# SobeyMIL/MVOC

Measured on AMD Instinct MI355X. Metric: UNet3D denoising steps/sec, 16x512^2 frames, inversion+compose, higher is better.
Workload: dtype f16

## Files before the change

### include/mvoc_hip.h

```cpp
#ifndef MVOC_HIP_H
#define MVOC_HIP_H

#include <stddef.h>
#include <stdint.h>

#ifdef __cplusplus
extern "C" {
#endif

#define MVOC_VERSION 100

int mvoc_version(void);
const char* mvoc_last_error(void);

enum { MVOC_A_PLAIN = 0, MVOC_A_CONV3X3 = 1, MVOC_A_TEMPORAL3 = 2 };
enum { MVOC_ACT_NONE = 0, MVOC_ACT_GEGLU = 1, MVOC_ACT_SILU = 2, MVOC_ACT_GELU = 3 };

typedef struct mvoc_gemm_desc {
  const void* a;
  const void* a2;
  const void* w;
  void* out;
  const void* bias;
  const void* rowadd;
  const void* resid;
  int64_t m, n, k;
  int32_t n_store;
  int32_t ldo, ldr, ld_rowadd, rowadd_div;
  int32_t a_mode;
  int32_t lda, lda2;
  int32_t c1;
  int32_t cin;
  int32_t nimg, hout, wout, hsrc, wsrc, stride, upsample, hup, wup;
  int32_t frames, hw;
  int32_t act;
  int32_t tile;
  int32_t split_k;
  void* workspace;
  size_t workspace_bytes;
  const void* ln_rowsum;
  const void* ln_bias;
  float ln_eps;
  int32_t pad_mode;
  const void* ln_stats;
  void* chan_sums;
  void* row_moments;
  int32_t row_moments_ld;
  int32_t concurrency;
  int32_t k_order;
} mvoc_gemm_desc;

int mvoc_gemm_f16(const mvoc_gemm_desc* d, void* stream);
int mvoc_gemm_chan_sums_written(void);
int mvoc_gemm_row_moments_written(void);
int mvoc_row_stats_from_moments_f32(const void* moments, int64_t rows, int32_t ld, int32_t n, int32_t tile_w, float eps,
                                    void* out_stats, void* stream);
size_t mvoc_gemm_workspace_bytes(int64_t m, int64_t n, int64_t k);

typedef struct mvoc_attn_desc {
  const void *q, *k, *v;
  void* out;
  int64_t q_bs, q_ts, k_bs, k_ts, v_bs, v_ts, o_bs, o_ts;
  int32_t nbatch, heads, tq, tk, kv_bdiv;
  int32_t head_dim, causal;
  float scale;
  const void* v2;
  void* out2;
  int32_t pipelined;
} mvoc_attn_desc;

int mvoc_flash_attn_f16(const mvoc_attn_desc* d, void* stream);
typedef struct mvoc_tattn_desc {
  const void *q, *k, *v;
  void* out;
  int64_t q_bs, q_ps, q_ts, k_bs, k_ps, k_ts, v_bs, v_ps, v_ts, o_bs, o_ps, o_ts;
  int32_t nsample, hw, heads, frames;
} mvoc_tattn_desc;
int mvoc_temporal_attn_f16(const mvoc_tattn_desc* d, void* stream);

typedef struct mvoc_xs_desc {
  const void* x;
  const void* wp;
  const void* resid;
  void* out;
  int64_t m;
  int32_t n, k, n_store, ldo, ldr, act, normalize;
  float ln_eps;
  int64_t wp_set_rows;
} mvoc_xs_desc;
int mvoc_xs_linear_f16(const mvoc_xs_desc* d, void* stream);


typedef struct mvoc_tfused_desc {
  const void* x;
  const void* wp;
  const void* ln_rowsum;
  const void* ln_bias;
  void* out;
  int32_t nsample, frames, hw, c, heads;
  float ln_eps;
} mvoc_tfused_desc;
int mvoc_temporal_qkv_attn_f16(const mvoc_tfused_desc* d, void* stream);

typedef struct mvoc_gn_desc {
  const void* x;
  const void* x2;
  const void* gamma;
  const void* beta;
  void* out;
  void* workspace;
  size_t workspace_bytes;
  int32_t nsample, rows_per_sample, c, c1, groups, silu;
  float eps;
  const void* chan_sums;
  const void* chan_sums2;
} mvoc_gn_desc;
size_t mvoc_groupnorm_workspace_bytes(int32_t nsample, int32_t rows_per_sample, int32_t c, int32_t groups);
int mvoc_groupnorm_f16(const mvoc_gn_desc* d, void* stream);
int mvoc_groupnorm_fold_xs_f16(const mvoc_gn_desc* d, const void* w, const void* bias, int32_t n, int32_t k, void* wp_sets,
                               void* stream);

int mvoc_groupnorm_moments_f16(const mvoc_gn_desc* d, void* moments, void* stream);
int mvoc_groupnorm_apply_moments_f16(const mvoc_gn_desc* d, const void* parts, int32_t nparts, void* stream);

int mvoc_row_stats_f16(const void* x, void* stats, int64_t rows, int32_t c, float eps, void* stream);

int mvoc_layernorm_f16(const void* x, const void* gamma, const void* beta, void* out, int64_t rows, int32_t c,
                       float eps, void* stream);

typedef struct mvoc_pnp_desc {
  void* x;
  void* x2;
  const void* masks;
  int64_t chunk_stride, f_stride, p_stride;
  int32_t nobj, frames, height, width, channels, mask_h, mask_w, base_chunk0;
  int32_t ndst;
} mvoc_pnp_desc;
int mvoc_pnp_blend_scatter_tokens(const mvoc_pnp_desc* d, void* stream);
int mvoc_pnp_blend_scatter_nchw(const mvoc_pnp_desc* d, void* stream);
int mvoc_pnp_blend_scatter_tokens_mapped(const mvoc_pnp_desc* d, int32_t nsrc, const int32_t* obj_chunk, void* stream);
int mvoc_pnp_blend_scatter_nchw_mapped(const mvoc_pnp_desc* d, int32_t nsrc, const int32_t* obj_chunk, void* stream);
int mvoc_pnp_blend_scatter_tokens_variants(const mvoc_pnp_desc* d, int32_t nsrc, const int32_t* obj_chunk, int32_t nvar,
                                           void* stream);
int mvoc_pnp_blend_scatter_nchw_variants(const mvoc_pnp_desc* d, int32_t nsrc, const int32_t* obj_chunk, int32_t nvar,
                                         void* stream);
int mvoc_pnp_blend_scatter_tokens_variants_sel(const mvoc_pnp_desc* d, int32_t nsrc, const int32_t* obj_chunk, int32_t nvar,
                                               uint32_t active, void* stream);
int mvoc_pnp_blend_scatter_nchw_variants_sel(const mvoc_pnp_desc* d, int32_t nsrc, const int32_t* obj_chunk, int32_t nvar,
                                             uint32_t active, void* stream);
int mvoc_pnp_blend_scatter_tokens_placed(const mvoc_pnp_desc* d, int32_t nsrc, const int32_t* obj_chunk, int32_t nvar,
                                         uint32_t active, const int32_t* place, void* stream);
int mvoc_pnp_blend_scatter_nchw_placed(const mvoc_pnp_desc* d, int32_t nsrc, const int32_t* obj_chunk, int32_t nvar,
                                       uint32_t active, const int32_t* place, void* stream);
int mvoc_pnp_blend_scatter_tokens_placed_variants(const mvoc_pnp_desc* d, int32_t nsrc, const int32_t* obj_chunk, int32_t nvar,
                                                  uint32_t active, const int32_t* place, void* stream);
int mvoc_pnp_blend_scatter_nchw_placed_variants(const mvoc_pnp_desc* d, int32_t nsrc, const int32_t* obj_chunk, int32_t nvar,
                                                uint32_t active, const int32_t* place, void* stream);
int mvoc_shift_planes_f16(const void* src, void* dst, int32_t nplane, int32_t frames, int32_t h, int32_t w,
                          const int32_t* offsets, void* stream);
int mvoc_pnp_blend_scatter_tokens_resampled(const mvoc_pnp_desc* d, int32_t nsrc, const int32_t* obj_chunk, int32_t nvar,
                                            uint32_t active, const int32_t* maps, void* stream);
int mvoc_pnp_blend_scatter_nchw_resampled(const mvoc_pnp_desc* d, int32_t nsrc, const int32_t* obj_chunk, int32_t nvar,
                                          uint32_t active, const int32_t* maps, void* stream);
int mvoc_pnp_blend_scatter_tokens_resampled_variants(const mvoc_pnp_desc* d, int32_t nsrc, const int32_t* obj_chunk, int32_t nvar,
                                                     uint32_t active, const int32_t* maps, void* stream);
int mvoc_pnp_blend_scatter_nchw_resampled_variants(const mvoc_pnp_desc* d, int32_t nsrc, const int32_t* obj_chunk, int32_t nvar,
                                                   uint32_t active, const int32_t* maps, void* stream);
int mvoc_gather_planes_f16(const void* src, void* dst, int32_t nplane, int32_t frames, int32_t h, int32_t w,
                           const int32_t* maps, void* stream);

int mvoc_ddim_step_f16(const void* x, const void* v_uncond, const void* v_cond, const float* coef_dev, void* out,
                       int64_t n, void* stream);
int mvoc_latent_fusion_f16(const void* latents, const void* bg, const void* objs, const void* masks, void* out,
                           int32_t nobj, int64_t n, double mix_ratio, int32_t obj_random_noise_fusion, void* stream);
int mvoc_ddim_step_variants_f16(const void* x, const void* v_uncond, const void* v_cond, const float* coef_dev, void* out,
                                int64_t n_per, int32_t nvar, void* stream);
int mvoc_latent_fusion_variants_f16(const void* latents, const void* bg, const void* objs, const void* masks, void* out,
                                    int32_t nobj, int64_t n_per, int32_t nvar, double mix_ratio,
                                    int32_t obj_random_noise_fusion, void* stream);

int mvoc_timestep_embedding_f16(const float* t_dev, int32_t nb, int32_t dim, void* out, void* stream);
int mvoc_act_f16(const void* x, void* out, int64_t n, int32_t act, void* stream);
int mvoc_add_f16(const void* a, const void* b, void* out, int64_t n, void* stream);
int mvoc_conv3x3_small_f16(const void* x, const void* w, const void* bias, void* out, int32_t nimg, int32_t h,
                           int32_t wd, int32_t cin, int32_t cout, int32_t stride, int32_t silu, void* stream);
int mvoc_adaptive_avgpool_f16(const void* x, void* out, int32_t nimg, int32_t h, int32_t w, int32_t c, int32_t oh,
                              int32_t ow, void* stream);
int mvoc_ncfhw_to_tokens_f16(const void* x, void* out, int32_t b, int32_t c, int32_t f, int32_t hw, int32_t ldo,
                             int32_t coff, void* stream);
int mvoc_tokens_to_ncfhw_f16(const void* x, void* out, int32_t b, int32_t c, int32_t f, int32_t hw, int32_t ld,
                             void* stream);
int mvoc_temporal_encoder4_f16(const void* x, const void* params, void* out, int32_t b, int32_t f, int32_t hw,
                               int32_t ldo, int32_t coff, void* stream);

int mvoc_conv1x1_small_f16(const void* x, const void* w, const void* bias, void* out, int64_t rows, int32_t cin,
                           int32_t cout, void* stream);
int mvoc_softmax_rows_f16(void* x, int64_t rows, int32_t cols, void* stream);
int mvoc_gaussian_sample_f16(const void* mean, const void* logvar, const void* noise, void* out, int64_t n, void* stream);
int mvoc_scale_f16(const void* x, void* out, int64_t n, double scale, void* stream);
int mvoc_image_to_tokens_f16(const void* x, void* out, int32_t n, int32_t c, int32_t hw, void* stream);
int mvoc_tokens_to_image_f16(const void* x, void* out, int32_t n, int32_t c, int32_t hw, int32_t ld, void* stream);

int mvoc_mask_resize_u8(const void* in, void* tmp, void* out, int32_t n, int32_t H, int32_t W, int32_t h, int32_t w,
                        const int32_t* bounds_h, const int32_t* kk_h, int32_t ksize_h, const int32_t* bounds_v,
                        const int32_t* kk_v, int32_t ksize_v, void* stream);
int mvoc_mask_finish(const void* v, void* float_mask, void* bool_mask, int64_t n, void* stream);

int mvoc_clip_patches_f16(const void* pixels, void* out, int32_t nimg, int32_t size, int32_t patch, int32_t kpad, void* stream);
int mvoc_clip_embed_f16(const void* table, const int32_t* ids, const void* cls, const void* pos, void* out, int64_t rows,
                        int32_t t, int32_t c, void* stream);

int mvoc_permute_rows_f16(const void* x, void* out, const int64_t* dims4, const int64_t* strides4, int32_t c, void* stream);
int mvoc_comm_unique_id(void* id128);
int mvoc_comm_init(const void* id128, int32_t rank, int32_t world, void** comm);
int mvoc_comm_destroy(void* comm);
int mvoc_allgather_frames(void* comm, const void* send, void* recv, size_t bytes_per_rank, void* stream);
int mvoc_alltoall_frames(void* comm, const void* send, void* recv, size_t bytes_per_peer, void* stream);

enum { MVOC_FAM_GEMM = 0, MVOC_FAM_FLASH = 1, MVOC_FAM_TATTN = 2, MVOC_FAM_GN = 3, MVOC_FAM_LN = 4, MVOC_FAM_PNP = 5,
       MVOC_FAM_MISC = 6, MVOC_FAM_TFUSED = 7, MVOC_FAM_COUNT = 8 };
int mvoc_prof_enable(int on);
int mvoc_prof_collect(double* ms_per_family, int64_t* launches_per_family, double* flops_or_bytes_per_family);
int mvoc_prof_reset(void);
int mvoc_delay_us(int64_t us, void* stream);

#ifdef __cplusplus
}
#endif
#endif
```

### mvoc_amd/_ffi.py

```python
import ctypes as C
import os

import torch

_HERE = os.path.dirname(os.path.abspath(__file__))
LIB_PATH = os.environ.get("MVOC_HIP_LIB") or os.path.join(_HERE, "libmvoc_hip.so")

ABI_VERSION = 100

A_PLAIN, A_CONV3X3, A_TEMPORAL3 = 0, 1, 2
ACT_NONE, ACT_GEGLU, ACT_SILU, ACT_GELU = 0, 1, 2, 3
FAMILIES = ("gemm", "flash_attn", "temporal_attn", "groupnorm", "layernorm", "pnp", "misc", "temporal_fused")

vp, i32, i64, f32, f64, sz = C.c_void_p, C.c_int32, C.c_int64, C.c_float, C.c_double, C.c_size_t


class GemmDesc(C.Structure):
    _fields_ = [("a", vp), ("a2", vp), ("w", vp), ("out", vp), ("bias", vp), ("rowadd", vp), ("resid", vp),
                ("m", i64), ("n", i64), ("k", i64), ("n_store", i32), ("ldo", i32), ("ldr", i32), ("ld_rowadd", i32),
                ("rowadd_div", i32), ("a_mode", i32), ("lda", i32), ("lda2", i32), ("c1", i32), ("cin", i32),
                ("nimg", i32), ("hout", i32), ("wout", i32), ("hsrc", i32), ("wsrc", i32), ("stride", i32),
                ("upsample", i32), ("hup", i32), ("wup", i32), ("frames", i32), ("hw", i32), ("act", i32), ("tile", i32),
                ("split_k", i32), ("workspace", vp), ("workspace_bytes", sz), ("ln_rowsum", vp), ("ln_bias", vp),
                ("ln_eps", f32), ("pad_mode", i32), ("ln_stats", vp), ("chan_sums", vp), ("row_moments", vp),
                ("row_moments_ld", i32), ("concurrency", i32), ("k_order", i32)]


class AttnDesc(C.Structure):
    _fields_ = [("q", vp), ("k", vp), ("v", vp), ("out", vp),
                ("q_bs", i64), ("q_ts", i64), ("k_bs", i64), ("k_ts", i64), ("v_bs", i64), ("v_ts", i64),
                ("o_bs", i64), ("o_ts", i64),
                ("nbatch", i32), ("heads", i32), ("tq", i32), ("tk", i32), ("kv_bdiv", i32),
                ("head_dim", i32), ("causal", i32), ("scale", C.c_float), ("v2", vp), ("out2", vp), ("pipelined", i32)]


class TAttnDesc(C.Structure):
    _fields_ = [("q", vp), ("k", vp), ("v", vp), ("out", vp),
                ("q_bs", i64), ("q_ps", i64), ("q_ts", i64), ("k_bs", i64), ("k_ps", i64), ("k_ts", i64),
                ("v_bs", i64), ("v_ps", i64), ("v_ts", i64), ("o_bs", i64), ("o_ps", i64), ("o_ts", i64),
                ("nsample", i32), ("hw", i32), ("heads", i32), ("frames", i32)]


class GnDesc(C.Structure):
    _fields_ = [("x", vp), ("x2", vp), ("gamma", vp), ("beta", vp), ("out", vp), ("workspace", vp),
                ("workspace_bytes", sz), ("nsample", i32), ("rows_per_sample", i32), ("c", i32), ("c1", i32),
                ("groups", i32), ("silu", i32), ("eps", f32), ("chan_sums", vp), ("chan_sums2", vp)]


class TFusedDesc(C.Structure):
    _fields_ = [("x", vp), ("wp", vp), ("ln_rowsum", vp), ("ln_bias", vp), ("out", vp), ("nsample", i32), ("frames", i32),
                ("hw", i32), ("c", i32), ("heads", i32), ("ln_eps", f32)]


class XsDesc(C.Structure):
    _fields_ = [("x", vp), ("wp", vp), ("resid", vp), ("out", vp), ("m", i64),
                ("n", i32), ("k", i32), ("n_store", i32), ("ldo", i32), ("ldr", i32), ("act", i32), ("normalize", i32),
                ("ln_eps", C.c_float), ("wp_set_rows", i64)]


class PnpDesc(C.Structure):
    _fields_ = [("x", vp), ("x2", vp), ("masks", vp), ("chunk_stride", i64), ("f_stride", i64), ("p_stride", i64),
                ("nobj", i32), ("frames", i32), ("height", i32), ("width", i32), ("channels", i32), ("mask_h", i32),
                ("mask_w", i32), ("base_chunk0", i32), ("ndst", i32)]


SIGNATURES = {
    "mvoc_version": (i32, []),
    "mvoc_last_error": (C.c_char_p, []),
    "mvoc_gemm_f16": (i32, [C.POINTER(GemmDesc), vp]),
    "mvoc_gemm_workspace_bytes": (sz, [i64, i64, i64]),
    "mvoc_gemm_chan_sums_written": (i32, []),
    "mvoc_gemm_row_moments_written": (i32, []),
    "mvoc_row_stats_from_moments_f32": (i32, [vp, i64, i32, i32, i32, f32, vp, vp]),
    "mvoc_flash_attn_f16": (i32, [C.POINTER(AttnDesc), vp]),
    "mvoc_temporal_attn_f16": (i32, [C.POINTER(TAttnDesc), vp]),
    "mvoc_temporal_qkv_attn_f16": (i32, [C.POINTER(TFusedDesc), vp]),
    "mvoc_xs_linear_f16": (i32, [C.POINTER(XsDesc), vp]),
    "mvoc_groupnorm_workspace_bytes": (sz, [i32, i32, i32, i32]),
    "mvoc_groupnorm_f16": (i32, [C.POINTER(GnDesc), vp]),
    "mvoc_groupnorm_fold_xs_f16": (i32, [C.POINTER(GnDesc), vp, vp, i32, i32, vp, vp]),
    "mvoc_groupnorm_moments_f16": (i32, [C.POINTER(GnDesc), vp, vp]),
    "mvoc_groupnorm_apply_moments_f16": (i32, [C.POINTER(GnDesc), vp, i32, vp]),
    "mvoc_layernorm_f16": (i32, [vp, vp, vp, vp, i64, i32, f32, vp]),
    "mvoc_row_stats_f16": (i32, [vp, vp, i64, i32, f32, vp]),
    "mvoc_pnp_blend_scatter_tokens": (i32, [C.POINTER(PnpDesc), vp]),
    "mvoc_pnp_blend_scatter_nchw": (i32, [C.POINTER(PnpDesc), vp]),
    "mvoc_pnp_blend_scatter_tokens_mapped": (i32, [C.POINTER(PnpDesc), i32, C.POINTER(i32), vp]),
    "mvoc_pnp_blend_scatter_nchw_mapped": (i32, [C.POINTER(PnpDesc), i32, C.POINTER(i32), vp]),
    "mvoc_pnp_blend_scatter_tokens_variants": (i32, [C.POINTER(PnpDesc), i32, C.POINTER(i32), i32, vp]),
    "mvoc_pnp_blend_scatter_nchw_variants": (i32, [C.POINTER(PnpDesc), i32, C.POINTER(i32), i32, vp]),
    "mvoc_pnp_blend_scatter_tokens_variants_sel": (i32, [C.POINTER(PnpDesc), i32, C.POINTER(i32), i32, C.c_uint32, vp]),
    "mvoc_pnp_blend_scatter_nchw_variants_sel": (i32, [C.POINTER(PnpDesc), i32, C.POINTER(i32), i32, C.c_uint32, vp]),
    "mvoc_pnp_blend_scatter_tokens_placed": (i32, [C.POINTER(PnpDesc), i32, C.POINTER(i32), i32, C.c_uint32, vp, vp]),
    "mvoc_pnp_blend_scatter_nchw_placed": (i32, [C.POINTER(PnpDesc), i32, C.POINTER(i32), i32, C.c_uint32, vp, vp]),
    "mvoc_pnp_blend_scatter_tokens_placed_variants": (i32, [C.POINTER(PnpDesc), i32, C.POINTER(i32), i32, C.c_uint32, vp, vp]),
    "mvoc_pnp_blend_scatter_nchw_placed_variants": (i32, [C.POINTER(PnpDesc), i32, C.POINTER(i32), i32, C.c_uint32, vp, vp]),
    "mvoc_shift_planes_f16": (i32, [vp, vp, i32, i32, i32, i32, vp, vp]),
    "mvoc_pnp_blend_scatter_tokens_resampled": (i32, [C.POINTER(PnpDesc), i32, C.POINTER(i32), i32, C.c_uint32, vp, vp]),
    "mvoc_pnp_blend_scatter_nchw_resampled": (i32, [C.POINTER(PnpDesc), i32, C.POINTER(i32), i32, C.c_uint32, vp, vp]),
    "mvoc_pnp_blend_scatter_tokens_resampled_variants": (i32, [C.POINTER(PnpDesc), i32, C.POINTER(i32), i32, C.c_uint32, vp, vp]),
    "mvoc_pnp_blend_scatter_nchw_resampled_variants": (i32, [C.POINTER(PnpDesc), i32, C.POINTER(i32), i32, C.c_uint32, vp, vp]),
    "mvoc_gather_planes_f16": (i32, [vp, vp, i32, i32, i32, i32, vp, vp]),
    "mvoc_ddim_step_f16": (i32, [vp, vp, vp, vp, vp, i64, vp]),
    "mvoc_latent_fusion_f16": (i32, [vp, vp, vp, vp, vp, i32, i64, f64, i32, vp]),
    "mvoc_ddim_step_variants_f16": (i32, [vp, vp, vp, vp, vp, i64, i32, vp]),
    "mvoc_latent_fusion_variants_f16": (i32, [vp, vp, vp, vp, vp, i32, i64, i32, f64, i32, vp]),
    "mvoc_timestep_embedding_f16": (i32, [vp, i32, i32, vp, vp]),
    "mvoc_act_f16": (i32, [vp, vp, i64, i32, vp]),
    "mvoc_add_f16": (i32, [vp, vp, vp, i64, vp]),
    "mvoc_conv3x3_small_f16": (i32, [vp, vp, vp, vp, i32, i32, i32, i32, i32, i32, i32, vp]),
    "mvoc_adaptive_avgpool_f16": (i32, [vp, vp, i32, i32, i32, i32, i32, i32, vp]),
    "mvoc_ncfhw_to_tokens_f16": (i32, [vp, vp, i32, i32, i32, i32, i32, i32, vp]),
    "mvoc_tokens_to_ncfhw_f16": (i32, [vp, vp, i32, i32, i32, i32, i32, vp]),
    "mvoc_temporal_encoder4_f16": (i32, [vp, vp, vp, i32, i32, i32, i32, i32, vp]),
    "mvoc_conv1x1_small_f16": (i32, [vp, vp, vp, vp, i64, i32, i32, vp]),
    "mvoc_softmax_rows_f16": (i32, [vp, i64, i32, vp]),
    "mvoc_gaussian_sample_f16": (i32, [vp, vp, vp, vp, i64, vp]),
    "mvoc_scale_f16": (i32, [vp, vp, i64, f64, vp]),
    "mvoc_image_to_tokens_f16": (i32, [vp, vp, i32, i32, i32, vp]),
    "mvoc_tokens_to_image_f16": (i32, [vp, vp, i32, i32, i32, i32, vp]),
    "mvoc_mask_resize_u8": (i32, [vp, vp, vp, i32, i32, i32, i32, i32, vp, vp, i32, vp, vp, i32, vp]),
    "mvoc_mask_finish": (i32, [vp, vp, vp, i64, vp]),
    "mvoc_permute_rows_f16": (i32, [vp, vp, C.POINTER(i64), C.POINTER(i64), i32, vp]),
    "mvoc_clip_patches_f16": (i32, [vp, vp, i32, i32, i32, i32, vp]),
    "mvoc_clip_embed_f16": (i32, [vp, vp, vp, vp, vp, i64, i32, i32, vp]),
    "mvoc_comm_unique_id": (i32, [vp]),
    "mvoc_comm_init": (i32, [vp, i32, i32, C.POINTER(vp)]),
    "mvoc_comm_destroy": (i32, [vp]),
    "mvoc_allgather_frames": (i32, [vp, vp, vp, sz, vp]),
    "mvoc_alltoall_frames": (i32, [vp, vp, vp, sz, vp]),
    "mvoc_prof_enable": (i32, [i32]),
    "mvoc_prof_collect": (i32, [C.POINTER(f64), C.POINTER(i64), C.POINTER(f64)]),
    "mvoc_prof_reset": (i32, []),
    "mvoc_delay_us": (i32, [i64, vp]),
}


def _load():
    if not os.path.exists(LIB_PATH):
        raise ImportError(
            f"{LIB_PATH} is missing: build it with `python -m mvoc_amd.build` (hipcc --offload-arch=gfx950). "
            "mvoc_amd has no CPU / PyTorch fallback path.")
    lib = C.CDLL(LIB_PATH)
    for name, (res, args) in SIGNATURES.items():
        fn = getattr(lib, name)
        fn.restype = res
        fn.argtypes = args
    if lib.mvoc_version() != ABI_VERSION:
        raise ImportError(f"{LIB_PATH} has mvoc_version() {lib.mvoc_version()}, these bindings need {ABI_VERSION}: rebuild it "
                          "with `python -m mvoc_amd.build`")
    return lib


lib = _load()


_DEBUG_SYNC = bool(os.environ.get("MVOC_DEBUG_SYNC"))


def check(rc, what=""):
    if rc != 0:
        raise RuntimeError(f"libmvoc_hip {what} failed ({rc}): {lib.mvoc_last_error().decode()}")
    if _DEBUG_SYNC:
        print(f"[mvoc] {what}", flush=True)
        torch.cuda.synchronize()
```

### mvoc_amd/csrc/xslin.hip

```cpp
#include <stdlib.h>

#include "common.h"

namespace {

struct XsArgs {
  const half_t* x;
  const half_t* wp;
  const half_t* resid;
  half_t* out;
  long M;
  int N, n_store, ldo, ldr, act, normalize;
  float eps;
  unsigned long long* stamps;
  int lab;
  long set_rows;
  long set_bytes;
};

#ifdef MVOC_PP_LAB
#define XS_STAMP(t) asm volatile("s_memtime %0\n\ts_waitcnt lgkmcnt(0)" : "=s"(t)::"memory")
#define XS_ACC(slot, a, b) (acc_t[slot] += (b) - (a))
#else
#define XS_STAMP(t) do { } while (0)
#define XS_ACC(slot, a, b) do { } while (0)
#endif

template <int N_>
__device__ __forceinline__ void xs_wait() {
  asm volatile("s_waitcnt vmcnt(%0)" ::"n"(N_) : "memory");
}
__device__ __forceinline__ void xs_wait_n(int n) {
  switch (n) {
    case 0: xs_wait<0>(); break;   case 1: xs_wait<1>(); break;   case 2: xs_wait<2>(); break;   case 3: xs_wait<3>(); break;
    case 4: xs_wait<4>(); break;   case 5: xs_wait<5>(); break;   case 6: xs_wait<6>(); break;   case 7: xs_wait<7>(); break;
    case 8: xs_wait<8>(); break;   case 9: xs_wait<9>(); break;   case 10: xs_wait<10>(); break; case 11: xs_wait<11>(); break;
    case 12: xs_wait<12>(); break; case 13: xs_wait<13>(); break; case 14: xs_wait<14>(); break; case 15: xs_wait<15>(); break;
    case 16: xs_wait<16>(); break; case 17: xs_wait<17>(); break; case 18: xs_wait<18>(); break; case 19: xs_wait<19>(); break;
    case 20: xs_wait<20>(); break; case 21: xs_wait<21>(); break; default: xs_wait<22>(); break;
  }
}

template <int NK, int RG, int ACT>
__global__ __launch_bounds__(256, 2) void xslin_kernel(const XsArgs p) {
  constexpr int NS = 3, NW = 4;
  constexpr int NP = NK + 1;
  constexpr int STAGE = NP * 1024;
  constexpr int K = NK * 16;
  constexpr int RBUF = 4096;
  __shared__ __attribute__((aligned(1024))) char smem[NS * STAGE + NW * RBUF];
  const int tid = threadIdx.x, lane = tid & 63;
  const int wave = __builtin_amdgcn_readfirstlane(tid >> 6);
  const int r = lane & 31, h = lane >> 5;
  long ms[RG];
#pragma unroll
  for (int g = 0; g < RG; ++g) {
    const long m = (long)blockIdx.x * (NW * 32 * RG) + wave * (32 * RG) + 32 * g + r;
    ms[g] = m < p.M ? m : p.M - 1;
  }

  const char* wp_set = reinterpret_cast<const char*>(p.wp) +
                       (p.set_rows > 0 ? ((long)blockIdx.x * (NW * 32 * RG) / p.set_rows) * p.set_bytes : 0);
  const int pw = (NP - wave + NW - 1) / NW;
  const int T = p.N / 32;
  auto issue = [&](int st) {
    const char* src = wp_set + (size_t)st * STAGE + lane * 16;
    char* dst = smem + (st % NS) * STAGE;
#pragma unroll
    for (int i = 0; i < (NP + NW - 1) / NW; ++i) {
      const int j = wave + NW * i;
      if (j < NP)
        __builtin_amdgcn_global_load_lds((const __attribute__((address_space(1))) void*)(src + j * 1024),
                                         (__attribute__((address_space(3))) void*)(dst + j * 1024), 16, 0, 0);
    }
  };
  char* resbuf = smem + NS * STAGE + wave * RBUF;
  auto res_slot = [&](int tile, int g, int j) -> char* {
    return resbuf + (RG == 1 ? (tile & 1) * 2048 : g * 2048) + j * 1024;
  };
  auto issue_resid = [&](int tile) {
#pragma unroll
    for (int g = 0; g < RG; ++g)
#pragma unroll
      for (int j = 0; j < 2; ++j) {
        int n = 32 * tile + 16 * j + 8 * h;
        n = n < p.n_store ? n : p.n_store - 8;
        __builtin_amdgcn_global_load_lds((const __attribute__((address_space(1))) void*)(p.resid + ms[g] * p.ldr + n),
                                         (__attribute__((address_space(3))) void*)res_slot(tile, g, j), 16, 0, 0);
      }
  };
  const int S = 2 * RG, R = p.resid ? 2 * RG : 0;
  constexpr bool GEGLU = ACT == MVOC_ACT_GEGLU;
  constexpr bool geglu = GEGLU;
  constexpr int PW_LO = NP / NW, PW_HI = (NP + NW - 1) / NW;
  auto wait_stage = [&](int st) {
    if (st >= 2 && st + 1 < T) {
      if (geglu) {
        if (pw == PW_HI) xs_wait<PW_HI + 2 * RG>(); else xs_wait<PW_LO + 2 * RG>();
      } else if (p.resid) {
        if (pw == PW_HI) xs_wait<PW_HI + 8 * RG>(); else xs_wait<PW_LO + 8 * RG>();
      } else {
        if (pw == PW_HI) xs_wait<PW_HI + 4 * RG>(); else xs_wait<PW_LO + 4 * RG>();
      }
      return;
    }
    const int dma_next = st + 1 < T ? pw : 0;
    int n;
    if (st == 0) n = dma_next;
    else if (geglu) n = dma_next + (st >= 2 ? S : 0);
    else n = dma_next + (st >= 2 ? 2 * (R + S) : R + S);
    xs_wait_n(n);
  };
  auto wait_resid = [&](int st) {
    if (RG == 1) xs_wait_n((st >= 1 ? S : 0) + (st + 2 < T ? pw : 0) + (st + 1 < T ? R : 0));
    else xs_wait_n(st >= 1 && st + 2 < T ? pw : 0);
  };

  half8_t xf[RG][NK];
#pragma unroll
  for (int g = 0; g < RG; ++g) {
    const half_t* xr = p.x + ms[g] * K + 8 * h;
#pragma unroll
    for (int s = 0; s < NK; ++s) xf[g][s] = *reinterpret_cast<const half8_t*>(xr + 16 * s);
  }
  if (p.resid) issue_resid(0);
  for (int st = 0; st < NS - 1 && st < T; ++st) issue(st);
  if (p.normalize) {
    const half2_t one2 = {(half_t)1.0f, (half_t)1.0f};
#pragma unroll
    for (int g = 0; g < RG; ++g) {
      float s1 = 0.f;
#pragma unroll
      for (int s = 0; s < NK; ++s)
#pragma unroll
        for (int e = 0; e < 4; ++e) {
          const half2_t v2 = {xf[g][s][2 * e], xf[g][s][2 * e + 1]};
          s1 = __builtin_amdgcn_fdot2(v2, one2, s1, false);
        }
      s1 += __shfl_xor(s1, 32);
      const float mu = s1 / (float)K;
      const half_t c16 = (half_t)mu;
      const half2_t c2 = {c16, c16};
      float t1 = 0.f, t2 = 0.f;
#pragma unroll
      for (int s = 0; s < NK; ++s)
#pragma unroll
        for (int e = 0; e < 4; ++e) {
          const half2_t v2 = {xf[g][s][2 * e], xf[g][s][2 * e + 1]};
          const half2_t d2 = v2 - c2;
          t1 = __builtin_amdgcn_fdot2(d2, one2, t1, false);
          t2 = __builtin_amdgcn_fdot2(d2, d2, t2, false);
        }
      t1 += __shfl_xor(t1, 32);
      t2 += __shfl_xor(t2, 32);
      const float dm = t1 / (float)K;
      const float rs = rsqrtf(fmaxf(t2 / (float)K - dm * dm, 0.f) + p.eps);
#pragma unroll
      for (int s = 0; s < NK; ++s)
#pragma unroll
        for (int e = 0; e < 8; ++e) xf[g][s][e] = (half_t)(((float)xf[g][s][e] - mu) * rs);
    }
  }

  int stage = 0;
  constexpr int PD = NK < 8 ? NK : (RG == 1 ? 8 : (GEGLU ? 2 : 4));
  const char* cslot = smem;
#ifdef MVOC_PP_LAB
  unsigned long long acc_t[6] = {0, 0, 0, 0, 0, 0}, ta = 0, tb = 0, tc = 0, td = 0, te = 0, tstart = 0;
  XS_STAMP(tstart);
  te = tstart;
#endif
  auto run_stage = [&](f32x16 (&acc)[RG]) {
    XS_STAMP(ta);
    XS_ACC(3, te, ta);
    wait_stage(stage);
    XS_STAMP(tb);
    XS_ACC(0, ta, tb);
    __builtin_amdgcn_sched_barrier(0);
    __builtin_amdgcn_s_barrier();
    __builtin_amdgcn_sched_barrier(0);
    XS_STAMP(tc);
    XS_ACC(1, tb, tc);
    if (stage + NS - 1 < T) issue(stage + NS - 1);
    if (RG == 1 && p.resid && stage + 1 < T) issue_resid(stage + 1);
    cslot = smem + (stage % NS) * STAGE;
    const char* wl = cslot + lane * 16;
    half8_t wf[PD];
#pragma unroll
    for (int i = 0; i < PD; ++i) wf[i] = *reinterpret_cast<const half8_t*>(wl + i * 1024);
    __builtin_amdgcn_sched_group_barrier(0x100, PD, 0);
#pragma unroll
    for (int s = 0; s < NK; ++s) {
#pragma unroll
      for (int g = 0; g < RG; ++g) acc[g] = __builtin_amdgcn_mfma_f32_32x32x16_f16(wf[s % PD], xf[g][s], acc[g], 0, 0, 0);
      if (s + PD < NK) wf[s % PD] = *reinterpret_cast<const half8_t*>(wl + (s + PD) * 1024);
      __builtin_amdgcn_sched_group_barrier(0x008, RG, 0);
      __builtin_amdgcn_sched_group_barrier(0x100, 1, 0);
    }
#ifdef MVOC_PP_LAB
    asm volatile("s_nop 0" ::"v"(acc[0][0]), "v"(acc[RG - 1][15]));
#endif
    XS_STAMP(te);
    XS_ACC(2, tc, te);
    ++stage;
  };
  auto cvec4 = [&](const char* slot, int c) -> f32x4 { return *reinterpret_cast<const f32x4*>(slot + NK * 1024 + c * 4); };
  auto store_tile = [&](unsigned (&pk)[4][2], int nout, int tile, int g) {
#pragma unroll
    for (int qq = 0; qq < 4; qq += 2)
#pragma unroll
      for (int w2 = 0; w2 < 2; ++w2) {
        const auto sw = __builtin_amdgcn_permlane32_swap(pk[qq][w2], pk[qq + 1][w2], false, false);
        pk[qq][w2] = sw[0];
        pk[qq + 1][w2] = sw[1];
      }
#pragma unroll
    for (int j = 0; j < 2; ++j) {
      const int n = nout + 16 * j + 8 * h;
      uint4 v = {pk[2 * j][0], pk[2 * j][1], pk[2 * j + 1][0], pk[2 * j + 1][1]};
      if (p.resid) {
        half8_t a = __builtin_bit_cast(half8_t, v);
        const half8_t b = *reinterpret_cast<const half8_t*>(res_slot(tile, g, j) + lane * 16);
#pragma unroll
        for (int e = 0; e < 8; ++e) a[e] = (half_t)((float)a[e] + (float)b[e]);
        v = __builtin_bit_cast(uint4, a);
      }
      if (n >= p.n_store) continue;
#ifdef MVOC_PP_LAB
      if (p.lab & 1) { asm volatile("" ::"v"(v.x), "v"(v.y), "v"(v.z), "v"(v.w)); continue; }
      if (p.lab & 2) {
        *reinterpret_cast<uint4*>(p.out + ((long)blockIdx.x * 1024 + (wave * 2 * RG + 2 * g + j)) * 512 + lane * 8 + (long)(nout / 32) * 0) = v;
        continue;
      }
#endif
      *reinterpret_cast<uint4*>(p.out + ms[g] * p.ldo + n) = v;
    }
  };

  if constexpr (GEGLU) {
    for (int t = 0; t + 1 < T; t += 2) {
      f32x16 acc[RG];
#pragma unroll
      for (int g = 0; g < RG; ++g)
#pragma unroll
        for (int e = 0; e < 16; ++e) acc[g][e] = 0.f;
      run_stage(acc);
      half2_t hv[RG][8];
#pragma unroll
      for (int q = 0; q < 4; ++q) {
        const f32x4 cvl = cvec4(cslot, 8 * q + 4 * h);
#pragma unroll
        for (int g = 0; g < RG; ++g) {
          hv[g][2 * q] = half2_t{(half_t)(acc[g][4 * q] + cvl[0]), (half_t)(acc[g][4 * q + 1] + cvl[1])};
          hv[g][2 * q + 1] = half2_t{(half_t)(acc[g][4 * q + 2] + cvl[2]), (half_t)(acc[g][4 * q + 3] + cvl[3])};
        }
      }
#pragma unroll
      for (int g = 0; g < RG; ++g)
#pragma unroll
        for (int e = 0; e < 16; ++e) acc[g][e] = 0.f;
      run_stage(acc);
#pragma unroll
      for (int g = 0; g < RG; ++g) {
        unsigned pk[4][2];
#pragma unroll
        for (int q = 0; q < 4; ++q) {
          const f32x4 cgt = cvec4(cslot, 8 * q + 4 * h);
          half_t o[4];
#pragma unroll
          for (int e = 0; e < 4; ++e) {
            const float gv = r16(acc[g][4 * q + e] + cgt[e]);
            o[e] = (half_t)((float)hv[g][2 * q + (e >> 1)][e & 1] * r16(gelu_fast_f(gv)));
          }
          const half2_t lo = {o[0], o[1]}, hi = {o[2], o[3]};
          pk[q][0] = __builtin_bit_cast(unsigned, lo);
          pk[q][1] = __builtin_bit_cast(unsigned, hi);
        }
        store_tile(pk, 16 * t, t + 1, g);
      }
    }
  } else {
    for (int t = 0; t < T; ++t) {
      f32x16 acc[RG];
#pragma unroll
      for (int g = 0; g < RG; ++g)
#pragma unroll
        for (int e = 0; e < 16; ++e) acc[g][e] = 0.f;
      run_stage(acc);
      if (p.resid) wait_resid(t);
#pragma unroll
      for (int g = 0; g < RG; ++g) {
        unsigned pk[4][2];
#pragma unroll
        for (int q = 0; q < 4; ++q) {
          const f32x4 cv = cvec4(cslot, 8 * q + 4 * h);
          half_t o[4];
#pragma unroll
          for (int e = 0; e < 4; ++e) {
            float v = r16(acc[g][4 * q + e] + cv[e]);
            if constexpr (ACT == MVOC_ACT_SILU) v = r16(silu_f(v));
            else if constexpr (ACT == MVOC_ACT_GELU) v = r16(gelu_fast_f(v));
            o[e] = (half_t)v;
          }
          const half2_t lo = {o[0], o[1]}, hi = {o[2], o[3]};
          pk[q][0] = __builtin_bit_cast(unsigned, lo);
          pk[q][1] = __builtin_bit_cast(unsigned, hi);
        }
        store_tile(pk, 32 * t, t, g);
      }
      if (RG == 2 && p.resid && t + 1 < T) {
        asm volatile("s_waitcnt lgkmcnt(0)" ::: "memory");
        issue_resid(t + 1);
      }
    }
  }
#ifdef MVOC_PP_LAB
  XS_STAMP(ta);
  XS_ACC(3, te, ta);
  if (p.stamps && blockIdx.x == 0 && wave == 0 && lane == 0) {
    for (int i = 0; i < 4; ++i) p.stamps[i] = acc_t[i];
    p.stamps[4] = ta - tstart;
    p.stamps[5] = (unsigned long long)T;
  }
#endif
}

}

extern "C" int mvoc_xs_linear_f16(const mvoc_xs_desc* d, void* stream) {
  MVOC_REQUIRE(d && d->x && d->wp && d->out, -1, "xs_linear: null operand");
  MVOC_REQUIRE(d->m > 0 && d->n > 0 && d->n % 32 == 0, -1, "xs_linear: m > 0, n %% 32 == 0");
  MVOC_REQUIRE(d->act >= MVOC_ACT_NONE && d->act <= MVOC_ACT_GELU, -1, "xs_linear: bad act %d", d->act);
  MVOC_REQUIRE(!(d->resid && d->act == MVOC_ACT_GEGLU), -2, "xs_linear: no residual with GEGLU");
  MVOC_REQUIRE(d->k == 64 || d->k == 128 || d->k == 320, -2, "xs_linear: k (%d) must be 64, 128 or 320", d->k);
  MVOC_REQUIRE(d->act != MVOC_ACT_GEGLU || d->n % 64 == 0, -2, "xs_linear: GEGLU needs n %% 64 == 0");
  const int ns = d->n_store > 0 ? d->n_store : (d->act == MVOC_ACT_GEGLU ? d->n / 2 : d->n);
  MVOC_REQUIRE(ns > (d->act == MVOC_ACT_GEGLU ? d->n / 2 : d->n) - 32, -2, "xs_linear: n_store may only trim the last 32-channel tile");
  MVOC_REQUIRE(ns % 8 == 0 && d->ldo % 8 == 0 && ((uintptr_t)d->out & 15) == 0 &&
                   (d->resid == nullptr || (d->ldr % 8 == 0 && ((uintptr_t)d->resid & 15) == 0)),
               -2, "xs_linear: outputs / residual must be 16-byte addressable per 8 channels");
  MVOC_REQUIRE(((uintptr_t)d->x & 15) == 0 && ((uintptr_t)d->wp & 15) == 0, -2,
               "xs_linear: x / wp must be 16-byte addressable (both are read in 16-byte pieces)");
  XsArgs a;
  a.x = (const half_t*)d->x; a.wp = (const half_t*)d->wp;
  a.resid = (const half_t*)d->resid; a.out = (half_t*)d->out;
  a.M = d->m; a.N = d->n; a.n_store = ns; a.ldo = d->ldo; a.ldr = d->ldr; a.act = d->act; a.normalize = d->normalize; a.eps = d->ln_eps;
  static const int force_rg = getenv("MVOC_XS_RG") ? atoi(getenv("MVOC_XS_RG")) : 0;
  const int rg = force_rg ? force_rg : (d->m >= 131072 && d->k == 320 ? 2 : 1);
  a.stamps = nullptr;
  a.lab = 0;
  a.set_rows = d->wp_set_rows;
  a.set_bytes = (long)(d->n / 32) * (d->k / 16 + 1) * 1024;
  MVOC_REQUIRE(d->wp_set_rows >= 0 && (d->wp_set_rows == 0 || (d->wp_set_rows % (128 * rg) == 0 && d->m % d->wp_set_rows == 0)), -2,
               "xs_linear: wp_set_rows (%ld) must be a multiple of the %d rows of a block and divide m", (long)d->wp_set_rows, 128 * rg);
#ifdef MVOC_PP_LAB
  if (const char* e = getenv("MVOC_XS_STAMPS")) a.stamps = (unsigned long long*)strtoull(e, nullptr, 10);
  a.lab = getenv("MVOC_XS_LAB") ? atoi(getenv("MVOC_XS_LAB")) : 0;
#endif
  const long nblk = (d->m + 128 * rg - 1) / (128 * rg);
  MVOC_REQUIRE(nblk < 0x7fffffffL, -2, "xs_linear: grid too large");
  hipStream_t s = (hipStream_t)stream;
  MvocProfScope prof(MVOC_FAM_GEMM, s, 2.0 * (double)d->m * d->n * d->k);
  const dim3 grid((unsigned)nblk), blk(256);
#define XS_LAUNCH(NK_, RG_)                                                                                        \
  do {                                                                                                             \
    if (d->act == MVOC_ACT_GEGLU) hipLaunchKernelGGL((xslin_kernel<NK_, RG_, MVOC_ACT_GEGLU>), grid, blk, 0, s, a);  \
    else if (d->act == MVOC_ACT_SILU) hipLaunchKernelGGL((xslin_kernel<NK_, RG_, MVOC_ACT_SILU>), grid, blk, 0, s, a); \
    else if (d->act == MVOC_ACT_GELU) hipLaunchKernelGGL((xslin_kernel<NK_, RG_, MVOC_ACT_GELU>), grid, blk, 0, s, a); \
    else hipLaunchKernelGGL((xslin_kernel<NK_, RG_, MVOC_ACT_NONE>), grid, blk, 0, s, a);                          \
  } while (0)
  if (d->k == 320 && rg == 2) XS_LAUNCH(20, 2);
  else if (d->k == 320) XS_LAUNCH(20, 1);
  else if (d->k == 128 && rg == 2) XS_LAUNCH(8, 2);
  else if (d->k == 128) XS_LAUNCH(8, 1);
  else if (rg == 2) XS_LAUNCH(4, 2);
  else XS_LAUNCH(4, 1);
#undef XS_LAUNCH
  return mvoc_check_launch("xslin_kernel");
}
```

Before: 24.96.

## Add software-pipelined xs_linear kernel overlapping epilogue with next tile's MFMAs

Adds a new xs_linear kernel for K=320 (plain or GEGLU epilogue) that interleaves each tile's epilogue (conversion, permlane swap, residual add, GELU gating, stores) into the MFMA loop of the following tile. It uses a three-stage LDS buffer for weights with explicit vmcnt waits, aiming to hide epilogue and store latency behind matrix work. It is enabled by default for eligible shapes, and the RG=2 heuristic now also requires n>320. This relies on hand-counted wait counts, and a mistake there could cause correctness risks or stalls.

```diff
diff --git a/include/mvoc_hip.h b/include/mvoc_hip.h
--- a/include/mvoc_hip.h
+++ b/include/mvoc_hip.h
@@ -89,6 +89,7 @@
   int64_t wp_set_rows;
 } mvoc_xs_desc;
 int mvoc_xs_linear_f16(const mvoc_xs_desc* d, void* stream);
+int mvoc_xs_force_form(int32_t rg, int32_t pipe);
 
 
 typedef struct mvoc_tfused_desc {
diff --git a/mvoc_amd/_ffi.py b/mvoc_amd/_ffi.py
--- a/mvoc_amd/_ffi.py
+++ b/mvoc_amd/_ffi.py
@@ -76,6 +76,7 @@
     "mvoc_temporal_attn_f16": (i32, [C.POINTER(TAttnDesc), vp]),
     "mvoc_temporal_qkv_attn_f16": (i32, [C.POINTER(TFusedDesc), vp]),
     "mvoc_xs_linear_f16": (i32, [C.POINTER(XsDesc), vp]),
+    "mvoc_xs_force_form": (i32, [i32, i32]),
     "mvoc_groupnorm_workspace_bytes": (sz, [i32, i32, i32, i32]),
     "mvoc_groupnorm_f16": (i32, [C.POINTER(GnDesc), vp]),
     "mvoc_groupnorm_fold_xs_f16": (i32, [C.POINTER(GnDesc), vp, vp, i32, i32, vp, vp]),
diff --git a/mvoc_amd/csrc/xslin.hip b/mvoc_amd/csrc/xslin.hip
--- a/mvoc_amd/csrc/xslin.hip
+++ b/mvoc_amd/csrc/xslin.hip
@@ -25,6 +25,9 @@
 #define XS_STAMP(t) do { } while (0)
 #define XS_ACC(slot, a, b) do { } while (0)
 #endif
+
+template <int V>
+struct xs_int { static constexpr int value = V; };
 
 template <int N_>
 __device__ __forceinline__ void xs_wait() {
@@ -325,6 +328,328 @@
 #endif
 }
 
+template <int NK, int RG, int ACT>
+__global__ __launch_bounds__(256, 2) void xslin_pipe_kernel(const XsArgs p) {
+  constexpr int NS = 3, NW = 4;
+  constexpr int NP = NK + 1;
+  constexpr int STAGE = NP * 1024;
+  constexpr int K = NK * 16;
+  constexpr int RBUF = 4096;
+  __shared__ __attribute__((aligned(1024))) char smem[NS * STAGE + NW * RBUF];
+  const int tid = threadIdx.x, lane = tid & 63;
+  const int wave = __builtin_amdgcn_readfirstlane(tid >> 6);
+  const int r = lane & 31, h = lane >> 5;
+  long ms[RG];
+#pragma unroll
+  for (int g = 0; g < RG; ++g) {
+    const long m = (long)blockIdx.x * (NW * 32 * RG) + wave * (32 * RG) + 32 * g + r;
+    ms[g] = m < p.M ? m : p.M - 1;
+  }
+
+  const char* wp_set = reinterpret_cast<const char*>(p.wp) +
+                       (p.set_rows > 0 ? ((long)blockIdx.x * (NW * 32 * RG) / p.set_rows) * p.set_bytes : 0);
+  const int pw = (NP - wave + NW - 1) / NW;
+  const int T = p.N / 32;
+  auto issue = [&](int st) {
+    const char* src = wp_set + (size_t)st * STAGE + lane * 16;
+    char* dst = smem + (st % NS) * STAGE;
+#pragma unroll
+    for (int i = 0; i < (NP + NW - 1) / NW; ++i) {
+      const int j = wave + NW * i;
+      if (j < NP)
+        __builtin_amdgcn_global_load_lds((const __attribute__((address_space(1))) void*)(src + j * 1024),
+                                         (__attribute__((address_space(3))) void*)(dst + j * 1024), 16, 0, 0);
+    }
+  };
+  char* resbuf = smem + NS * STAGE + wave * RBUF;
+  auto res_slot = [&](int tile, int g, int j) -> char* {
+    return resbuf + (RG == 1 ? (tile & 1) * 2048 : g * 2048) + j * 1024;
+  };
+  auto issue_resid_g = [&](int tile, int g) __attribute__((always_inline)) {
+#pragma unroll
+    for (int j = 0; j < 2; ++j) {
+      int n = 32 * tile + 16 * j + 8 * h;
+      n = n < p.n_store ? n : p.n_store - 8;
+      __builtin_amdgcn_global_load_lds((const __attribute__((address_space(1))) void*)(p.resid + ms[g] * p.ldr + n),
+                                       (__attribute__((address_space(3))) void*)res_slot(tile, g, j), 16, 0, 0);
+    }
+  };
+  auto issue_resid = [&](int tile) {
+#pragma unroll
+    for (int g = 0; g < RG; ++g) issue_resid_g(tile, g);
+  };
+  constexpr bool GEGLU = ACT == MVOC_ACT_GEGLU;
+  constexpr bool geglu = GEGLU;
+  constexpr int PW_LO = NP / NW, PW_HI = (NP + NW - 1) / NW;
+
+  half8_t xf[RG][NK];
+#pragma unroll
+  for (int g = 0; g < RG; ++g) {
+    const half_t* xr = p.x + ms[g] * K + 8 * h;
+#pragma unroll
+    for (int s = 0; s < NK; ++s) xf[g][s] = *reinterpret_cast<const half8_t*>(xr + 16 * s);
+  }
+  if (p.resid) issue_resid(0);
+  for (int st = 0; st < NS - 1 && st < T; ++st) issue(st);
+  if (p.normalize) {
+    const half2_t one2 = {(half_t)1.0f, (half_t)1.0f};
+#pragma unroll
+    for (int g = 0; g < RG; ++g) {
+      float s1 = 0.f;
+#pragma unroll
+      for (int s = 0; s < NK; ++s)
+#pragma unroll
+        for (int e = 0; e < 4; ++e) {
+          const half2_t v2 = {xf[g][s][2 * e], xf[g][s][2 * e + 1]};
+          s1 = __builtin_amdgcn_fdot2(v2, one2, s1, false);
+        }
+      s1 += __shfl_xor(s1, 32);
+      const float mu = s1 / (float)K;
+      const half_t c16 = (half_t)mu;
+      const half2_t c2 = {c16, c16};
+      float t1 = 0.f, t2 = 0.f;
+#pragma unroll
+      for (int s = 0; s < NK; ++s)
+#pragma unroll
+        for (int e = 0; e < 4; ++e) {
+          const half2_t v2 = {xf[g][s][2 * e], xf[g][s][2 * e + 1]};
+          const half2_t d2 = v2 - c2;
+          t1 = __builtin_amdgcn_fdot2(d2, one2, t1, false);
+          t2 = __builtin_amdgcn_fdot2(d2, d2, t2, false);
+        }
+      t1 += __shfl_xor(t1, 32);
+      t2 += __shfl_xor(t2, 32);
+      const float dm = t1 / (float)K;
+      const float rs = rsqrtf(fmaxf(t2 / (float)K - dm * dm, 0.f) + p.eps);
+#pragma unroll
+      for (int s = 0; s < NK; ++s)
+#pragma unroll
+        for (int e = 0; e < 8; ++e) xf[g][s][e] = (half_t)(((float)xf[g][s][e] - mu) * rs);
+    }
+  }
+
+  constexpr int PD = RG == 1 ? 8 : 4;
+  auto cvec4 = [&](const char* slot, int c) -> f32x4 { return *reinterpret_cast<const f32x4*>(slot + NK * 1024 + c * 4); };
+  auto swap_pair = [&](unsigned (&pk)[4][2], int qq) __attribute__((always_inline)) {
+#pragma unroll
+    for (int w2 = 0; w2 < 2; ++w2) {
+      const auto sw = __builtin_amdgcn_permlane32_swap(pk[qq][w2], pk[qq + 1][w2], false, false);
+      pk[qq][w2] = sw[0];
+      pk[qq + 1][w2] = sw[1];
+    }
+  };
+  auto resid_piece = [&](int tile, int g, int j) __attribute__((always_inline)) -> half8_t {
+    return *reinterpret_cast<const half8_t*>(res_slot(tile, g, j) + lane * 16);
+  };
+  auto store_piece = [&](unsigned (&pk)[4][2], int nout, int g, int j, bool use_resid, const half8_t b, bool check_n) __attribute__((always_inline)) {
+    const int n = nout + 16 * j + 8 * h;
+    uint4 v = {pk[2 * j][0], pk[2 * j][1], pk[2 * j + 1][0], pk[2 * j + 1][1]};
+    if (use_resid) {
+      half8_t a = __builtin_bit_cast(half8_t, v);
+#pragma unroll
+      for (int e = 0; e < 8; ++e) a[e] = (half_t)((float)a[e] + (float)b[e]);
+      v = __builtin_bit_cast(uint4, a);
+    }
+    if (check_n && n >= p.n_store) return;
+    *reinterpret_cast<uint4*>(p.out + ms[g] * p.ldo + n) = v;
+  };
+  static_assert(NK == 20 && (ACT == MVOC_ACT_NONE || (GEGLU && RG == 1)), "pipelined form: K = 320, plain epilogue, or GEGLU with one row group");
+  static_assert(2 * PW_LO >= 4 + PW_LO, "the first residual waits count on the prologue's DMA being newer than residual(0)");
+  auto wait_stage_p = [&](int t) __attribute__((always_inline)) {
+    if (t >= 4 && t + 1 < T) {
+      if (geglu) {
+        if (pw == PW_HI) xs_wait<PW_HI + 2 * RG>(); else xs_wait<PW_LO + 2 * RG>();
+      } else if (p.resid) {
+        if (pw == PW_HI) xs_wait<PW_HI + 8 * RG>(); else xs_wait<PW_LO + 8 * RG>();
+      } else {
+        if (pw == PW_HI) xs_wait<PW_HI + 4 * RG>(); else xs_wait<PW_LO + 4 * RG>();
+      }
+      return;
+    }
+    const int dma_next = t + 1 < T ? pw : 0;
+    const int epis = RG == 1 ? (t >= 3 ? 2 : t == 2 ? 1 : 0) : (t >= 3 ? 4 : t == 2 ? 3 : t);
+    if (geglu) xs_wait_n(dma_next + (t >= 4 ? 2 : t == 3 ? 1 : 0));
+    else xs_wait_n(dma_next + epis * (p.resid ? 4 : 2));
+  };
+  auto head = [&](int t) __attribute__((always_inline)) {
+    wait_stage_p(t);
+    asm volatile("s_waitcnt lgkmcnt(0)" ::: "memory");
+    __builtin_amdgcn_sched_barrier(0);
+    __builtin_amdgcn_s_barrier();
+    __builtin_amdgcn_sched_barrier(0);
+    if (t + 2 < T) issue(t + 2);
+  };
+  auto pass = [&](int t, auto gtag, f32x16& acc, auto between) __attribute__((always_inline)) {
+    constexpr int G = decltype(gtag)::value;
+    const char* wl = smem + __builtin_amdgcn_readfirstlane((t % NS) * STAGE) + lane * 16;
+#pragma unroll
+    for (int e = 0; e < 16; ++e) acc[e] = 0.f;
+    half8_t wf[PD];
+#pragma unroll
+    for (int i = 0; i < PD; ++i) wf[i] = *reinterpret_cast<const half8_t*>(wl + i * 1024);
+    __builtin_amdgcn_sched_barrier(0);
+#pragma unroll
+    for (int s = 0; s < NK; ++s) {
+      acc = __builtin_amdgcn_mfma_f32_32x32x16_f16(wf[s % PD], xf[G][s], acc, 0, 0, 0);
+      if (s + PD < NK) wf[s % PD] = *reinterpret_cast<const half8_t*>(wl + (s + PD) * 1024);
+      between(s);
+      __builtin_amdgcn_sched_barrier(0);
+    }
+  };
+  auto nothing = [](int) {};
+  auto add_consts = [&](int t, f32x16& acc) __attribute__((always_inline)) {
+    const char* slot = smem + __builtin_amdgcn_readfirstlane((t % NS) * STAGE);
+#pragma unroll
+    for (int q = 0; q < 4; ++q) {
+      const f32x4 cv = cvec4(slot, 8 * q + 4 * h);
+#pragma unroll
+      for (int e = 0; e < 4; ++e) acc[4 * q + e] = acc[4 * q + e] + cv[e];
+    }
+  };
+  unsigned pk[4][2];
+  if constexpr (GEGLU) {
+    half2_t hva[8], hvb[8];
+    f32x16 accv, gta, gtb;
+    auto epi_piece = [&](int s, int half, int tp, f32x16& pg, half2_t (&phv)[8], bool check_n) __attribute__((always_inline)) {
+      if (s < 16 && (s & 1)) {
+        const int i = 8 * half + (s >> 1), q = i >> 2, e = i & 3;
+        const float gv = r16(pg[i]);
+        float ge = gelu_fast_f(gv);
+        asm("" : "+v"(ge));
+        const half_t o = (half_t)((float)phv[2 * q + (e >> 1)][e & 1] * r16(ge));
+        half2_t w = __builtin_bit_cast(half2_t, pk[q][e >> 1]);
+        w[e & 1] = o;
+        pk[q][e >> 1] = __builtin_bit_cast(unsigned, w);
+      }
+      if (s == 17) {
+        swap_pair(pk, 2 * half);
+        store_piece(pk, 16 * tp, 0, half, false, half8_t{}, check_n);
+      }
+    };
+    auto pair = [&](int t, f32x16& g, half2_t (&hv)[8], f32x16& pg, half2_t (&phv)[8], bool has_prev) __attribute__((always_inline)) {
+      head(t);
+      if (has_prev) {
+#pragma unroll
+        for (int q = 0; q < 4; ++q) pk[q][0] = pk[q][1] = 0u;
+        pass(t, xs_int<0>{}, accv, [&](int s) { epi_piece(s, 0, t - 2, pg, phv, false); });
+      } else {
+        pass(t, xs_int<0>{}, accv, nothing);
+      }
+      add_consts(t, accv);
+#pragma unroll
+      for (int q = 0; q < 4; ++q) {
+        hv[2 * q] = half2_t{(half_t)accv[4 * q], (half_t)accv[4 * q + 1]};
+        hv[2 * q + 1] = half2_t{(half_t)accv[4 * q + 2], (half_t)accv[4 * q + 3]};
+      }
+      head(t + 1);
+      if (has_prev) pass(t + 1, xs_int<0>{}, g, [&](int s) { epi_piece(s, 1, t - 2, pg, phv, false); });
+      else pass(t + 1, xs_int<0>{}, g, nothing);
+      add_consts(t + 1, g);
+    };
+    const int P = T >> 1;
+    pair(0, gta, hva, gtb, hvb, false);
+    for (int u = 1; u < P; u += 2) {
+      pair(2 * u, gtb, hvb, gta, hva, true);
+      if (u + 1 < P) pair(2 * u + 2, gta, hva, gtb, hvb, true);
+    }
+#pragma unroll
+    for (int q = 0; q < 4; ++q) pk[q][0] = pk[q][1] = 0u;
+    if (P & 1) {
+#pragma unroll
+      for (int s = 0; s < 2 * NK; ++s) epi_piece(s % NK, s / NK, T - 2, gta, hva, true);
+    } else {
+#pragma unroll
+      for (int s = 0; s < 2 * NK; ++s) epi_piece(s % NK, s / NK, T - 2, gtb, hvb, true);
+    }
+  } else {
+    half8_t rb[2];
+    constexpr int WS = 4, ST0 = 8, STD = 8;
+    static_assert(ST0 - 1 > WS && ST0 + STD < NK, "every piece has its step");
+    auto epi_piece = [&](int s, int tile, int g, f32x16& pacc, bool use_resid, bool dn, bool check_n) __attribute__((always_inline)) {
+      if (s == 0) {
+#pragma unroll
+        for (int q = 0; q < 4; ++q) {
+          const half2_t lo = {(half_t)pacc[4 * q], (half_t)pacc[4 * q + 1]}, hi = {(half_t)pacc[4 * q + 2], (half_t)pacc[4 * q + 3]};
+          pk[q][0] = __builtin_bit_cast(unsigned, lo);
+          pk[q][1] = __builtin_bit_cast(unsigned, hi);
+        }
+        swap_pair(pk, 0);
+        swap_pair(pk, 2);
+      }
+      if (s == WS && use_resid) { if (dn) xs_wait<4 + PW_LO>(); else xs_wait<4>(); }
+#pragma unroll
+      for (int j = 0; j < 2; ++j) {
+        if (s == ST0 + STD * j - 1 && use_resid) rb[j] = resid_piece(tile, g, j);
+        if (s == ST0 + STD * j) store_piece(pk, 32 * tile, g, j, use_resid, rb[j], check_n);
+      }
+    };
+    auto epi_last = [&](int g, f32x16& pacc) __attribute__((always_inline)) {
+      if (p.resid) xs_wait<0>();
+#pragma unroll
+      for (int s = 0; s < NK; ++s) epi_piece(s, T - 1, g, pacc, p.resid != nullptr, false, true);
+    };
+    f32x16 acca, accb;
+    if constexpr (RG == 1) {
+      auto stage = [&](int t, f32x16& acc, f32x16& pacc, bool use_resid, bool dn) __attribute__((always_inline)) {
+        head(t);
+        if (use_resid) issue_resid(t);
+        pass(t, xs_int<0>{}, acc, [&](int s) { epi_piece(s, t - 1, 0, pacc, use_resid, dn, false); });
+        add_consts(t, acc);
+      };
+      head(0);
+      pass(0, xs_int<0>{}, acca, nothing);
+      add_consts(0, acca);
+      if (p.resid) {
+        for (int t = 1; t < T; t += 2) {
+          if (t + 2 < T) stage(t, accb, acca, true, true); else stage(t, accb, acca, true, false);
+          if (t + 1 < T) { if (t + 3 < T) stage(t + 1, acca, accb, true, true); else stage(t + 1, acca, accb, true, false); }
+        }
+      } else {
+        for (int t = 1; t < T; t += 2) {
+          stage(t, accb, acca, false, false);
+          if (t + 1 < T) stage(t + 1, acca, accb, false, false);
+        }
+      }
+      epi_last(0, (T & 1) ? acca : accb);
+    } else {
+      auto stage = [&](int t, bool first, bool use_resid, bool dn) __attribute__((always_inline)) {
+        head(t);
+        if (first) pass(t, xs_int<0>{}, acca, nothing);
+        else pass(t, xs_int<0>{}, acca, [&](int s) { epi_piece(s, t - 1, 1, accb, use_resid, dn, false); });
+        if (use_resid && !first) {
+          asm volatile("s_waitcnt lgkmcnt(0)" ::: "memory");
+          issue_resid_g(t, 1);
+        }
+        add_consts(t, acca);
+        pass(t, xs_int<1>{}, accb, [&](int s) { epi_piece(s, t, 0, acca, use_resid, dn, t + 1 == T); });
+        if (use_resid && t + 1 < T) {
+          asm volatile("s_waitcnt lgkmcnt(0)" ::: "memory");
+          issue_resid_g(t + 1, 0);
+        }
+        add_consts(t, accb);
+      };
+      if (p.resid) {
+        if (2 < T) stage(0, true, true, true); else stage(0, true, true, false);
+        for (int t = 1; t < T; ++t) { if (t + 2 < T) stage(t, false, true, true); else stage(t, false, true, false); }
+      } else {
+        stage(0, true, false, false);
+        for (int t = 1; t < T; ++t) stage(t, false, false, false);
+      }
+      epi_last(1, accb);
+    }
+  }
+}
+
+}
+
+static int xs_force_rg = getenv("MVOC_XS_RG") ? atoi(getenv("MVOC_XS_RG")) : 0;
+static int xs_force_pipe = getenv("MVOC_XS_PIPE") ? atoi(getenv("MVOC_XS_PIPE")) : -1;
+
+extern "C" int mvoc_xs_force_form(int rg, int pipe) {
+  MVOC_REQUIRE(rg >= 0 && rg <= 2 && pipe >= -1 && pipe <= 1, -1, "xs_force_form: rg in 0..2, pipe in -1..1");
+  xs_force_rg = rg;
+  xs_force_pipe = pipe;
+  return 0;
 }
 
 extern "C" int mvoc_xs_linear_f16(const mvoc_xs_desc* d, void* stream) {
@@ -345,8 +670,9 @@
   a.x = (const half_t*)d->x; a.wp = (const half_t*)d->wp;
   a.resid = (const half_t*)d->resid; a.out = (half_t*)d->out;
   a.M = d->m; a.N = d->n; a.n_store = ns; a.ldo = d->ldo; a.ldr = d->ldr; a.act = d->act; a.normalize = d->normalize; a.eps = d->ln_eps;
-  static const int force_rg = getenv("MVOC_XS_RG") ? atoi(getenv("MVOC_XS_RG")) : 0;
-  const int rg = force_rg ? force_rg : (d->m >= 131072 && d->k == 320 ? 2 : 1);
+  const int rg = xs_force_rg ? xs_force_rg : (d->m >= 131072 && d->k == 320 && d->n > 320 ? 2 : 1);
+  const bool pipe_able = d->k == 320 && (d->act == MVOC_ACT_NONE || (d->act == MVOC_ACT_GEGLU && rg == 1));
+  const bool pipe = pipe_able && (xs_force_pipe >= 0 ? xs_force_pipe != 0 : true);
   a.stamps = nullptr;
   a.lab = 0;
   a.set_rows = d->wp_set_rows;
@@ -369,7 +695,10 @@
     else if (d->act == MVOC_ACT_GELU) hipLaunchKernelGGL((xslin_kernel<NK_, RG_, MVOC_ACT_GELU>), grid, blk, 0, s, a); \
     else hipLaunchKernelGGL((xslin_kernel<NK_, RG_, MVOC_ACT_NONE>), grid, blk, 0, s, a);                          \
   } while (0)
-  if (d->k == 320 && rg == 2) XS_LAUNCH(20, 2);
+  if (pipe && d->act == MVOC_ACT_GEGLU) hipLaunchKernelGGL((xslin_pipe_kernel<20, 1, MVOC_ACT_GEGLU>), grid, blk, 0, s, a);
+  else if (pipe && rg == 2) hipLaunchKernelGGL((xslin_pipe_kernel<20, 2, MVOC_ACT_NONE>), grid, blk, 0, s, a);
+  else if (pipe) hipLaunchKernelGGL((xslin_pipe_kernel<20, 1, MVOC_ACT_NONE>), grid, blk, 0, s, a);
+  else if (d->k == 320 && rg == 2) XS_LAUNCH(20, 2);
   else if (d->k == 320) XS_LAUNCH(20, 1);
   else if (d->k == 128 && rg == 2) XS_LAUNCH(8, 2);
   else if (d->k == 128) XS_LAUNCH(8, 1);
```

Measured after the change: 24.99 (median of 5 runs). Within noise of the previous version (+0.1%).
